# DanEngelbrecht/longtail

Hardware: AMD Instinct MI355X
Metric: ingest GB/s (chunk+hash+compress) (higher is better)
Workload: dtype u8/u32

## Files before the change

longtail_amd/csrc/k_blake3.hip:

```cpp
#include "lthip_internal.h"

#include <stdlib.h>

namespace
{

enum
{
    F_CHUNK_START = 1,
    F_CHUNK_END = 2,
    F_PARENT = 4,
    F_ROOT = 8
};

#define B3_IV0 0x6A09E667u
#define B3_IV1 0xBB67AE85u
#define B3_IV2 0x3C6EF372u
#define B3_IV3 0xA54FF53Au
#define B3_IV4 0x510E527Fu
#define B3_IV5 0x9B05688Cu
#define B3_IV6 0x1F83D9ABu
#define B3_IV7 0x5BE0CD19u

__device__ __forceinline__ uint32_t rotr32(uint32_t x, uint32_t r) { return __builtin_amdgcn_alignbit(x, x, r); }

__device__ __forceinline__ void b3_g(uint32_t& a, uint32_t& b, uint32_t& c, uint32_t& d, uint32_t mx, uint32_t my)
{
    a = a + b + mx;
    d = rotr32(d ^ a, 16);
    c = c + d;
    b = rotr32(b ^ c, 12);
    a = a + b + my;
    d = rotr32(d ^ a, 8);
    c = c + d;
    b = rotr32(b ^ c, 7);
}

#define B3_ROUND(m0, m1, m2, m3, m4, m5, m6, m7, m8, m9, m10, m11, m12, m13, m14, m15) \
    b3_g(s0, s4, s8, s12, m0, m1);                                                      \
    b3_g(s1, s5, s9, s13, m2, m3);                                                      \
    b3_g(s2, s6, s10, s14, m4, m5);                                                     \
    b3_g(s3, s7, s11, s15, m6, m7);                                                     \
    b3_g(s0, s5, s10, s15, m8, m9);                                                     \
    b3_g(s1, s6, s11, s12, m10, m11);                                                   \
    b3_g(s2, s7, s8, s13, m12, m13);                                                    \
    b3_g(s3, s4, s9, s14, m14, m15);

__device__ __forceinline__ void b3_compress(uint32_t (&cv)[8], const uint32_t (&m)[16], uint32_t counter_lo,
                                            uint32_t block_len, uint32_t flags)
{
    uint32_t s0 = cv[0], s1 = cv[1], s2 = cv[2], s3 = cv[3], s4 = cv[4], s5 = cv[5], s6 = cv[6], s7 = cv[7];
    uint32_t s8 = B3_IV0, s9 = B3_IV1, s10 = B3_IV2, s11 = B3_IV3;
    uint32_t s12 = counter_lo, s13 = 0u, s14 = block_len, s15 = flags;
    B3_ROUND(m[0], m[1], m[2], m[3], m[4], m[5], m[6], m[7], m[8], m[9], m[10], m[11], m[12], m[13], m[14], m[15])
    B3_ROUND(m[2], m[6], m[3], m[10], m[7], m[0], m[4], m[13], m[1], m[11], m[12], m[5], m[9], m[14], m[15], m[8])
    B3_ROUND(m[3], m[4], m[10], m[12], m[13], m[2], m[7], m[14], m[6], m[5], m[9], m[0], m[11], m[15], m[8], m[1])
    B3_ROUND(m[10], m[7], m[12], m[9], m[14], m[3], m[13], m[15], m[4], m[0], m[11], m[2], m[5], m[8], m[1], m[6])
    B3_ROUND(m[12], m[13], m[9], m[11], m[15], m[10], m[14], m[8], m[7], m[2], m[5], m[3], m[0], m[1], m[6], m[4])
    B3_ROUND(m[9], m[14], m[11], m[5], m[8], m[12], m[15], m[1], m[13], m[3], m[0], m[10], m[2], m[6], m[4], m[7])
    B3_ROUND(m[11], m[15], m[5], m[0], m[1], m[9], m[8], m[6], m[14], m[10], m[2], m[12], m[3], m[4], m[7], m[13])
    cv[0] = s0 ^ s8;
    cv[1] = s1 ^ s9;
    cv[2] = s2 ^ s10;
    cv[3] = s3 ^ s11;
    cv[4] = s4 ^ s12;
    cv[5] = s5 ^ s13;
    cv[6] = s6 ^ s14;
    cv[7] = s7 ^ s15;
}

typedef uint32_t u32x4_a4 __attribute__((ext_vector_type(4), aligned(4)));

__device__ __forceinline__ uint32_t leaves_of(uint32_t len) { return len ? (len + 1023u) >> 10 : 1u; }

__global__ void k_leaf_counts(const uint32_t* __restrict__ lens, uint64_t bound, const uint32_t* __restrict__ n_dev,
                              uint32_t* __restrict__ counts)
{
    uint64_t i = (uint64_t)blockIdx.x * blockDim.x + threadIdx.x;
    uint64_t n = n_dev ? (*n_dev < bound ? *n_dev : bound) : bound;
    if (i < n)
        counts[i] = leaves_of(lens[i]);
}

#ifndef LTHIP_B3_PW
#define LTHIP_B3_PW 1024
#endif
constexpr int PW = LTHIP_B3_PW;
constexpr int PW_MAXN = 256;
constexpr int PW_SLOTS = PW + PW_MAXN;
#ifndef LTHIP_B3_PW_THREADS
#define LTHIP_B3_PW_THREADS 512
#endif
constexpr int PW_THREADS = LTHIP_B3_PW_THREADS;

__global__ __launch_bounds__(256) void k_blake3_leaves(const uint8_t* __restrict__ data,
                                                       const uint64_t* __restrict__ offsets,
                                                       const uint32_t* __restrict__ lens,
                                                       const uint32_t* __restrict__ leaf_prefix,
                                                       uint64_t count_bound, const uint32_t* __restrict__ n_dev,
                                                       uint32_t* __restrict__ cvs, uint32_t* __restrict__ win_first)
{
    const uint32_t count = (uint32_t)(n_dev ? (*n_dev < count_bound ? *n_dev : count_bound) : count_bound);
    const uint32_t total = leaf_prefix[count];
    const uint64_t g64 = (uint64_t)blockIdx.x * blockDim.x + threadIdx.x;
    if (g64 >= total)
        return;
    const uint32_t g = (uint32_t)g64;
    uint32_t lo = 0, hi = count;
    while (hi - lo > 1)
    {
        const uint32_t mid = lo + ((hi - lo) >> 1);
        if (leaf_prefix[mid] <= g)
            lo = mid;
        else
            hi = mid;
    }
    const uint32_t c = lo;
    const uint32_t first = leaf_prefix[c];
    const uint32_t k = g - first;
    if (win_first && (g & (uint32_t)(PW - 1)) == 0u)
        win_first[g / (uint32_t)PW] = k == 0u ? c : c + 1u;
    const uint32_t rlen = lens[c];
    const uint32_t nleaf = leaves_of(rlen);
    const uint32_t llen = rlen - (k << 10) < 1024u ? rlen - (k << 10) : 1024u;
    const uint8_t* p = data + offsets[c] + ((uint64_t)k << 10);
    const uint32_t root = nleaf == 1u ? (uint32_t)F_ROOT : 0u;

    const uint32_t mis = (uint32_t)((uintptr_t)p & 3u);
    const uint32_t sh = mis * 8u;
    const uint32_t* q = reinterpret_cast<const uint32_t*>(p - mis);

    uint32_t cv[8] = {B3_IV0, B3_IV1, B3_IV2, B3_IV3, B3_IV4, B3_IV5, B3_IV6, B3_IV7};
    const uint32_t nblocks = llen ? (llen + 63u) >> 6 : 1u;

    for (uint32_t b = 0; b + 1 < nblocks; ++b)
    {
        const uint32_t* src = q + b * 16u;
        uint32_t w[17];
        const u32x4_a4 v0 = *reinterpret_cast<const u32x4_a4*>(src);
        const u32x4_a4 v1 = *reinterpret_cast<const u32x4_a4*>(src + 4);
        const u32x4_a4 v2 = *reinterpret_cast<const u32x4_a4*>(src + 8);
        const u32x4_a4 v3 = *reinterpret_cast<const u32x4_a4*>(src + 12);
        w[0] = v0.x; w[1] = v0.y; w[2] = v0.z; w[3] = v0.w;
        w[4] = v1.x; w[5] = v1.y; w[6] = v1.z; w[7] = v1.w;
        w[8] = v2.x; w[9] = v2.y; w[10] = v2.z; w[11] = v2.w;
        w[12] = v3.x; w[13] = v3.y; w[14] = v3.z; w[15] = v3.w;
        w[16] = mis ? src[16] : 0u;
        uint32_t m[16];
#pragma unroll
        for (int i = 0; i < 16; ++i)
            m[i] = __builtin_amdgcn_alignbit(w[i + 1], w[i], sh);
        b3_compress(cv, m, k, 64u, b == 0 ? (uint32_t)F_CHUNK_START : 0u);
    }
    {
        const uint32_t b = nblocks - 1u;
        const uint32_t bl = llen - b * 64u;
        const uint32_t* src = q + b * 16u;
        const uint32_t nd = bl ? (mis + bl + 3u) >> 2 : 0u;
        uint32_t w[17];
#pragma unroll
        for (int i = 0; i < 17; ++i)
            w[i] = (uint32_t)i < nd ? src[i] : 0u;
        uint32_t m[16];
#pragma unroll
        for (int i = 0; i < 16; ++i)
        {
            uint32_t v = __builtin_amdgcn_alignbit(w[i + 1], w[i], sh);
            const int rem = (int)bl - 4 * i;
            if (rem <= 0)
                v = 0u;
            else if (rem < 4)
                v &= (1u << (8 * rem)) - 1u;
            m[i] = v;
        }
        uint32_t fl = (uint32_t)F_CHUNK_END | root;
        if (b == 0)
            fl |= (uint32_t)F_CHUNK_START;
        b3_compress(cv, m, k, bl, fl);
    }
    uint4* out = reinterpret_cast<uint4*>(cvs + (uint64_t)g * 8u);
    out[0] = make_uint4(cv[0], cv[1], cv[2], cv[3]);
    out[1] = make_uint4(cv[4], cv[5], cv[6], cv[7]);
}

__device__ __forceinline__ void b3_parent(uint32_t* __restrict__ left, const uint32_t* __restrict__ right, uint32_t flags)
{
    uint32_t m[16];
    const uint4 a0 = reinterpret_cast<const uint4*>(left)[0], a1 = reinterpret_cast<const uint4*>(left)[1];
    const uint4 b0 = reinterpret_cast<const uint4*>(right)[0], b1 = reinterpret_cast<const uint4*>(right)[1];
    m[0] = a0.x; m[1] = a0.y; m[2] = a0.z; m[3] = a0.w; m[4] = a1.x; m[5] = a1.y; m[6] = a1.z; m[7] = a1.w;
    m[8] = b0.x; m[9] = b0.y; m[10] = b0.z; m[11] = b0.w; m[12] = b1.x; m[13] = b1.y; m[14] = b1.z; m[15] = b1.w;
    uint32_t cv[8] = {B3_IV0, B3_IV1, B3_IV2, B3_IV3, B3_IV4, B3_IV5, B3_IV6, B3_IV7};
    b3_compress(cv, m, 0u, 64u, flags);
    reinterpret_cast<uint4*>(left)[0] = make_uint4(cv[0], cv[1], cv[2], cv[3]);
    reinterpret_cast<uint4*>(left)[1] = make_uint4(cv[4], cv[5], cv[6], cv[7]);
}

#ifdef LTHIP_ABLATIONS
#include "ablations/k_blake3_parents_small.inc"
#endif

constexpr uint32_t B3_ONE_PITCH = 1024u + 4u;
__global__ __launch_bounds__(64) void k_blake3_one(const uint8_t* __restrict__ in, uint32_t len, uint64_t* __restrict__ out)
{
    extern __shared__ __attribute__((aligned(16))) uint32_t s_one[];
    uint32_t* s_cv = s_one;
    uint32_t* s_in = s_one + 64 * 8;
    const uint32_t lane = threadIdx.x;
    const uint32_t nleaf = leaves_of(len);
    {
        const uint32_t nvec = (((uintptr_t)in & 15u) == 0u) ? len >> 4 : 0u;
        const uint4* in4 = reinterpret_cast<const uint4*>(in);
        for (uint32_t v0 = 0; v0 < nvec; v0 += 64u * 8u)
        {
            uint4 q[8];
#pragma unroll
            for (int u = 0; u < 8; ++u)
            {
                const uint32_t v = v0 + (uint32_t)u * 64u + lane;
                q[u] = v < nvec ? in4[v] : make_uint4(0, 0, 0, 0);
            }
#pragma unroll
            for (int u = 0; u < 8; ++u)
            {
                const uint32_t v = v0 + (uint32_t)u * 64u + lane;
                if (v < nvec)
                {
                    uint32_t* d = s_in + (v >> 6) * (B3_ONE_PITCH / 4u) + (v & 63u) * 4u;
                    d[0] = q[u].x;
                    d[1] = q[u].y;
                    d[2] = q[u].z;
                    d[3] = q[u].w;
                }
            }
        }
        for (uint32_t j = (nvec << 4) + lane; j < len; j += 64u)
            reinterpret_cast<uint8_t*>(s_in)[(j >> 10) * B3_ONE_PITCH + (j & 1023u)] = in[j];
    }
    __syncthreads();
    if (lane < nleaf)
    {
        const uint32_t llen = len - (lane << 10) < 1024u ? len - (lane << 10) : 1024u;
        const uint32_t* pw = s_in + lane * (B3_ONE_PITCH / 4u);
        const uint8_t* p = reinterpret_cast<const uint8_t*>(pw);
        const uint32_t nblocks = llen ? (llen + 63u) >> 6 : 1u;
        uint32_t cv[8] = {B3_IV0, B3_IV1, B3_IV2, B3_IV3, B3_IV4, B3_IV5, B3_IV6, B3_IV7};
        for (uint32_t b = 0; b < nblocks; ++b)
        {
            const uint32_t bl = llen - b * 64u < 64u ? llen - b * 64u : 64u;
            uint32_t m[16];
            if (bl == 64u)
            {
#pragma unroll
                for (int i = 0; i < 16; ++i)
                    m[i] = pw[b * 16u + (uint32_t)i];
            }
            else
            {
#pragma unroll
                for (int i = 0; i < 16; ++i)
                    m[i] = 0u;
                for (uint32_t j = 0; j < bl; ++j)
                    m[j >> 2] |= (uint32_t)p[b * 64u + j] << (8u * (j & 3u));
            }
            uint32_t fl = b == 0 ? (uint32_t)F_CHUNK_START : 0u;
            if (b + 1 == nblocks)
                fl |= (uint32_t)F_CHUNK_END | (nleaf == 1u ? (uint32_t)F_ROOT : 0u);
            b3_compress(cv, m, lane, bl, fl);
        }
#pragma unroll
        for (int i = 0; i < 8; ++i)
            s_cv[lane * 8 + i] = cv[i];
    }
    __syncthreads();
    for (uint32_t stride = 1; stride < nleaf; stride <<= 1)
    {
        const uint32_t last = (stride << 1) >= nleaf;
        const uint32_t k = lane * (stride << 1);
        if (k + stride < nleaf)
            b3_parent(s_cv + k * 8u, s_cv + (k + stride) * 8u, (uint32_t)F_PARENT | (last ? (uint32_t)F_ROOT : 0u));
        __syncthreads();
    }
    if (lane == 0)
        *out = (uint64_t)s_cv[0] | ((uint64_t)s_cv[1] << 32);
}

constexpr int B3S_LEAVES = 1024;

__global__ __launch_bounds__(B3S_LEAVES) void k_blake3_stream_batch(const uint8_t* __restrict__ data, uint32_t leaf0,
                                                                      uint32_t* __restrict__ stack, uint32_t depth_in, uint32_t merges)
{
    __shared__ uint32_t s_cv[B3S_LEAVES * 8];
    const uint32_t t = threadIdx.x;
    {
        const uint32_t* p = reinterpret_cast<const uint32_t*>(data) + (size_t)t * 256u;
        uint32_t cv[8] = {B3_IV0, B3_IV1, B3_IV2, B3_IV3, B3_IV4, B3_IV5, B3_IV6, B3_IV7};
        for (uint32_t b = 0; b < 16u; ++b)
        {
            uint32_t m[16];
            const uint4* q = reinterpret_cast<const uint4*>(p + b * 16u);
            const uint4 v0 = q[0], v1 = q[1], v2 = q[2], v3 = q[3];
            m[0] = v0.x; m[1] = v0.y; m[2] = v0.z; m[3] = v0.w; m[4] = v1.x; m[5] = v1.y; m[6] = v1.z; m[7] = v1.w;
            m[8] = v2.x; m[9] = v2.y; m[10] = v2.z; m[11] = v2.w; m[12] = v3.x; m[13] = v3.y; m[14] = v3.z; m[15] = v3.w;
            b3_compress(cv, m, leaf0 + t, 64u, (b == 0 ? (uint32_t)F_CHUNK_START : 0u) | (b == 15u ? (uint32_t)F_CHUNK_END : 0u));
        }
#pragma unroll
        for (int i = 0; i < 8; ++i)
            s_cv[t * 8 + i] = cv[i];
    }
    __syncthreads();
    for (uint32_t stride = 1; stride < (uint32_t)B3S_LEAVES; stride <<= 1)
    {
        if ((t & (2u * stride - 1u)) == 0u)
            b3_parent(s_cv + t * 8u, s_cv + (t + stride) * 8u, (uint32_t)F_PARENT);
        __syncthreads();
    }
    if (t == 0)
    {
        uint32_t depth = depth_in;
        for (int i = 0; i < 8; ++i)
            stack[depth * 8u + i] = s_cv[i];
        ++depth;
        for (uint32_t m = 0; m < merges; ++m)
        {
            b3_parent(stack + (depth - 2u) * 8u, stack + (depth - 1u) * 8u, (uint32_t)F_PARENT);
            --depth;
        }
    }
}

__global__ __launch_bounds__(B3S_LEAVES) void k_blake3_stream_final(const uint8_t* __restrict__ tail, uint32_t tail_len, uint32_t leaf0,
                                                                      const uint32_t* __restrict__ stack, uint32_t depth_in,
                                                                      uint64_t* __restrict__ out)
{
    __shared__ uint32_t s_cv[B3S_LEAVES * 8];
    __shared__ uint32_t s_stack[64 * 8];
    const uint32_t t = threadIdx.x;
    const uint32_t nleaf = tail_len ? (tail_len + 1023u) >> 10 : (leaf0 == 0u ? 1u : 0u);
    const bool single = leaf0 == 0u && nleaf == 1u;
    if (t < nleaf)
    {
        const uint32_t llen = tail_len - (t << 10) < 1024u ? tail_len - (t << 10) : 1024u;
        const uint8_t* p = tail + ((size_t)t << 10);
        const uint32_t nblocks = llen ? (llen + 63u) >> 6 : 1u;
        uint32_t cv[8] = {B3_IV0, B3_IV1, B3_IV2, B3_IV3, B3_IV4, B3_IV5, B3_IV6, B3_IV7};
        for (uint32_t b = 0; b < nblocks; ++b)
        {
            const uint32_t bl = llen - b * 64u < 64u ? llen - b * 64u : 64u;
            uint32_t m[16];
#pragma unroll
            for (int i = 0; i < 16; ++i)
                m[i] = 0u;
            for (uint32_t j = 0; j < bl; ++j)
                m[j >> 2] |= (uint32_t)p[b * 64u + j] << (8u * (j & 3u));
            uint32_t fl = b == 0 ? (uint32_t)F_CHUNK_START : 0u;
            if (b + 1 == nblocks)
                fl |= (uint32_t)F_CHUNK_END | (single ? (uint32_t)F_ROOT : 0u);
            b3_compress(cv, m, leaf0 + t, bl, fl);
        }
#pragma unroll
        for (int i = 0; i < 8; ++i)
            s_cv[t * 8 + i] = cv[i];
    }
    for (uint32_t i = t; i < depth_in * 8u; i += (uint32_t)B3S_LEAVES)
        s_stack[i] = stack[i];
    __syncthreads();
    if (t != 0)
        return;
    if (single)
    {
        *out = (uint64_t)s_cv[0] | ((uint64_t)s_cv[1] << 32);
        return;
    }
    uint32_t depth = depth_in;
    for (uint32_t j = 0; j + 1 < nleaf; ++j)
    {
        for (int i = 0; i < 8; ++i)
            s_stack[depth * 8u + i] = s_cv[j * 8u + i];
        ++depth;
        uint32_t cnt = leaf0 + j + 1u;
        while ((cnt & 1u) == 0u)
        {
            b3_parent(s_stack + (depth - 2u) * 8u, s_stack + (depth - 1u) * 8u, (uint32_t)F_PARENT);
            --depth;
            cnt >>= 1;
        }
    }
    uint32_t* cur = s_cv + (nleaf - 1u) * 8u;
    while (depth > 0u)
    {
        uint32_t* left = s_stack + (depth - 1u) * 8u;
        b3_parent(left, cur, (uint32_t)F_PARENT | (depth == 1u ? (uint32_t)F_ROOT : 0u));
        cur = left;
        --depth;
    }
    *out = (uint64_t)cur[0] | ((uint64_t)cur[1] << 32);
}

__global__ __launch_bounds__(PW_THREADS) void k_blake3_parents_window(const uint32_t* __restrict__ leaf_prefix, uint64_t count_bound,
                                                               const uint32_t* __restrict__ n_dev, const uint32_t* __restrict__ cvs,
                                                               const uint32_t* __restrict__ win_first, uint64_t* __restrict__ hashes)
{
    __shared__ uint4 s_cv[PW_SLOTS * 2];
    __shared__ uint32_t s_info[PW_SLOTS];
    __shared__ uint16_t s_list[PW_SLOTS / 2 + 64];
    __shared__ uint32_t s_cnt, s_maxn;
    const uint32_t count = (uint32_t)(n_dev ? (*n_dev < count_bound ? *n_dev : count_bound) : count_bound);
    const uint32_t total = leaf_prefix[count];
    const uint64_t w0 = (uint64_t)blockIdx.x * PW;
    if (w0 >= total)
        return;
    const int tid = threadIdx.x;
    const int lane = tid & 63;
    const uint32_t c_lo = win_first[blockIdx.x];
    const uint32_t c_hi = w0 + PW >= total ? count : win_first[blockIdx.x + 1u];
    const uint32_t nch = c_hi - c_lo;
    if (nch == 0)
        return;
    const uint32_t wbase = leaf_prefix[c_lo];
    const uint32_t nslots = leaf_prefix[c_hi] - wbase;
    if (tid == 0)
    {
        s_cnt = 0;
        s_maxn = 0;
    }
    {
        const uint4* g = reinterpret_cast<const uint4*>(cvs) + (uint64_t)wbase * 2u;
        for (uint32_t v = tid; v < nslots * 2u; v += PW_THREADS)
            s_cv[v] = g[v];
    }
    __syncthreads();
    if (nch * 8u < nslots)
    {
        for (uint32_t j = tid >> 6; j < nch; j += PW_THREADS / 64)
        {
            const uint32_t p0 = leaf_prefix[c_lo + j], n = leaf_prefix[c_lo + j + 1] - p0;
            for (uint32_t k = lane; k < n; k += 64)
                s_info[p0 - wbase + k] = k | (n << 16);
            if (lane == 0)
                atomicMax(&s_maxn, n);
        }
    }
    else
    {
        for (uint32_t j = tid; j < nch; j += PW_THREADS)
        {
            const uint32_t p0 = leaf_prefix[c_lo + j], n = leaf_prefix[c_lo + j + 1] - p0;
            for (uint32_t k = 0; k < n; ++k)
                s_info[p0 - wbase + k] = k | (n << 16);
            atomicMax(&s_maxn, n);
        }
    }
    __syncthreads();
    const uint32_t maxn = s_maxn;
    uint32_t rot = blockIdx.x;
    for (uint32_t st = 1; st < maxn; st <<= 1, ++rot)
    {
        for (uint32_t s0 = 0; s0 < nslots; s0 += PW_THREADS)
        {
            const uint32_t sl = s0 + (uint32_t)tid;
            const uint32_t info = sl < nslots ? s_info[sl] : 0u;
            const uint32_t k = info & 0xFFFFu, n = info >> 16;
            const bool is = (k & ((st << 1) - 1u)) == 0u && k + st < n;
            const uint64_t mask = __builtin_amdgcn_ballot_w64(is);
            uint32_t base = 0;
            if (lane == 0 && mask)
                base = atomicAdd(&s_cnt, (uint32_t)__builtin_popcountll(mask));
            base = __builtin_amdgcn_readfirstlane(base);
            if (is)
                s_list[base + (uint32_t)__builtin_popcountll(mask & ((1ull << lane) - 1ull))] = (uint16_t)sl;
        }
        __syncthreads();
        const uint32_t nm = s_cnt;
        for (uint32_t mi = ((uint32_t)tid + 64u * rot) & (uint32_t)(PW_THREADS - 1); mi < nm; mi += PW_THREADS)
        {
            const uint32_t sl = s_list[mi];
            const uint32_t n = s_info[sl] >> 16;
            const uint4 a0 = s_cv[2u * sl], a1 = s_cv[2u * sl + 1u];
            const uint4 b0 = s_cv[2u * (sl + st)], b1 = s_cv[2u * (sl + st) + 1u];
            uint32_t m[16] = {a0.x, a0.y, a0.z, a0.w, a1.x, a1.y, a1.z, a1.w, b0.x, b0.y, b0.z, b0.w, b1.x, b1.y, b1.z, b1.w};
            uint32_t cv[8] = {B3_IV0, B3_IV1, B3_IV2, B3_IV3, B3_IV4, B3_IV5, B3_IV6, B3_IV7};
            b3_compress(cv, m, 0u, 64u, (uint32_t)F_PARENT | ((st << 1) >= n ? (uint32_t)F_ROOT : 0u));
            s_cv[2u * sl] = make_uint4(cv[0], cv[1], cv[2], cv[3]);
            s_cv[2u * sl + 1u] = make_uint4(cv[4], cv[5], cv[6], cv[7]);
        }
        __syncthreads();
        if (tid == 0)
            s_cnt = 0;
        __syncthreads();
    }
    for (uint32_t j = tid; j < nch; j += PW_THREADS)
    {
        const uint4 r = s_cv[2u * (leaf_prefix[c_lo + j] - wbase)];
        hashes[c_lo + j] = (uint64_t)r.x | ((uint64_t)r.y << 32);
    }
}

__global__ __launch_bounds__(256) void k_blake3_parents_level(const uint32_t* __restrict__ leaf_prefix, uint32_t count,
                                                              uint32_t stride, uint32_t* __restrict__ cvs)
{
    const uint32_t total = leaf_prefix[count];
    const uint64_t g64 = (uint64_t)blockIdx.x * blockDim.x + threadIdx.x;
    if (g64 >= total)
        return;
    const uint32_t g = (uint32_t)g64;
    uint32_t lo = 0, hi = count;
    while (hi - lo > 1)
    {
        const uint32_t mid = lo + ((hi - lo) >> 1);
        if (leaf_prefix[mid] <= g)
            lo = mid;
        else
            hi = mid;
    }
    const uint32_t slot0 = leaf_prefix[lo];
    const uint32_t n = leaf_prefix[lo + 1] - slot0;
    const uint32_t k = g - slot0;
    if ((k & ((stride << 1) - 1u)) != 0u || k + stride >= n)
        return;
    const uint32_t last = (stride << 1) >= n;
    b3_parent(cvs + (uint64_t)g * 8u, cvs + (uint64_t)(g + stride) * 8u, (uint32_t)F_PARENT | (last ? (uint32_t)F_ROOT : 0u));
}

__global__ void k_blake3_emit(const uint32_t* __restrict__ leaf_prefix, uint32_t count, const uint32_t* __restrict__ cvs,
                              uint64_t* __restrict__ hashes)
{
    const uint64_t c = (uint64_t)blockIdx.x * blockDim.x + threadIdx.x;
    if (c >= count)
        return;
    const uint32_t* base = cvs + (uint64_t)leaf_prefix[c] * 8u;
    hashes[c] = (uint64_t)base[0] | ((uint64_t)base[1] << 32);
}

}

int lthip_launch_blake3(lthip_ctx* ctx, const uint8_t* d_data, const uint64_t* d_offsets, const uint32_t* d_lens,
                        const uint32_t* d_count, uint64_t count_bound, uint64_t leaf_bound, uint64_t max_len,
                        uint64_t* d_hashes)
{
    if (count_bound == 0)
        return 0;
    void *lc, *lp, *cv;
    int err;
    if ((err = lthip_scratch(ctx, S_LEAF_COUNT, (count_bound + 1) * 4, &lc)))
        return err;
    if ((err = lthip_scratch(ctx, S_LEAF_PREFIX, (count_bound + 1) * 4, &lp)))
        return err;
    {
        LaunchTimer t(ctx, LTHIP_K_COMPACT);
        hipLaunchKernelGGL(k_leaf_counts, dim3((uint32_t)div_up_u64(count_bound, 256)), dim3(256), 0, ctx->stream, d_lens,
                           count_bound, d_count, (uint32_t*)lc);
        LTHIP_LAUNCH_CHECK(ctx);
    }
    if ((err = lthip_exclusive_scan_u32(ctx, (const uint32_t*)lc, (uint32_t*)lp, count_bound, d_count, LTHIP_K_COMPACT)))
        return err;

    const bool small_trees = max_len != 0 && max_len <= 256u * 1024u;
    uint32_t host_count = 0;
    if (leaf_bound == 0 || !small_trees)
    {
        if (d_count)
        {
            LTHIP_CHECK(ctx, hipMemcpyAsync(&host_count, d_count, 4, hipMemcpyDeviceToHost, ctx->stream));
            LTHIP_CHECK(ctx, lthip_stream_wait(ctx));
            if (host_count > count_bound)
                host_count = (uint32_t)count_bound;
        }
        else
            host_count = (uint32_t)count_bound;
        uint32_t total = 0;
        LTHIP_CHECK(ctx, hipMemcpyAsync(&total, (const uint32_t*)lp + host_count, 4, hipMemcpyDeviceToHost, ctx->stream));
        LTHIP_CHECK(ctx, lthip_stream_wait(ctx));
        leaf_bound = total;
        if (host_count == 0)
            return 0;
    }
    if (leaf_bound == 0)
        return 0;
    if (leaf_bound > 0xFFFFFFF0ull)
        return lthip_fail(ctx, EINVAL, "blake3", "too many leaves in one batch");
    if ((err = lthip_scratch(ctx, S_CV, leaf_bound * 32, &cv)))
        return err;
    void* wf = nullptr;
    if (small_trees && (err = lthip_scratch(ctx, S_B3_WINDOWS, (leaf_bound / PW + 2) * 4, &wf)))
        return err;
    {
        LaunchTimer t(ctx, LTHIP_K_B3_LEAF);
        LTHIP_ABLATION_ENV(env_pad, "LTHIP_B3_PAD_LDS");
        const int pad_lds = env_pad.get() > 0 ? env_pad.get() : 0;
        hipLaunchKernelGGL(k_blake3_leaves, dim3((uint32_t)div_up_u64(leaf_bound, 256)), dim3(256), (size_t)pad_lds, ctx->stream, d_data,
                           d_offsets, d_lens, (const uint32_t*)lp, count_bound, d_count, (uint32_t*)cv, (uint32_t*)wf);
        LTHIP_LAUNCH_CHECK(ctx);
    }
    if (small_trees)
    {
        LaunchTimer t(ctx, LTHIP_K_B3_PARENT);
#ifdef LTHIP_ABLATIONS
        LTHIP_ABLATION_ENV(env_serial, "LTHIP_B3_SERIAL_PARENTS");
        if (env_serial.get() >= 0)
            hipLaunchKernelGGL(k_blake3_parents_small, dim3((uint32_t)div_up_u64(count_bound, 256)), dim3(256), 0, ctx->stream,
                               d_lens, (const uint32_t*)lp, count_bound, d_count, (uint32_t*)cv, d_hashes);
        else
#endif
            hipLaunchKernelGGL(k_blake3_parents_window, dim3((uint32_t)div_up_u64(leaf_bound, PW)), dim3(PW_THREADS), 0, ctx->stream,
                               (const uint32_t*)lp, count_bound, d_count, (const uint32_t*)cv, (const uint32_t*)wf, d_hashes);
        LTHIP_LAUNCH_CHECK(ctx);
    }
    else
    {
        LaunchTimer t(ctx, LTHIP_K_B3_PARENT);
        uint64_t max_leaves = max_len ? div_up_u64(max_len, 1024) : (1ull << 22);
        for (uint64_t stride = 1; stride < max_leaves; stride <<= 1)
            hipLaunchKernelGGL(k_blake3_parents_level, dim3((uint32_t)div_up_u64(leaf_bound, 256)), dim3(256), 0,
                               ctx->stream, (const uint32_t*)lp, host_count, (uint32_t)stride, (uint32_t*)cv);
        hipLaunchKernelGGL(k_blake3_emit, dim3((uint32_t)div_up_u64(host_count, 256)), dim3(256), 0, ctx->stream,
                           (const uint32_t*)lp, host_count, (const uint32_t*)cv, d_hashes);
        LTHIP_LAUNCH_CHECK(ctx);
    }
    return 0;
}

int lthip_launch_blake3_one(lthip_ctx* ctx, const void* in, uint32_t len, uint64_t* out)
{
    if (len > 65536u)
        return lthip_fail(ctx, EINVAL, "blake3_one", "input above 64 KiB");
    LaunchTimer t(ctx, LTHIP_K_B3_LEAF);
    const size_t lds = 64 * 8 * 4 + (size_t)(len ? (len + 1023u) >> 10 : 1u) * B3_ONE_PITCH;
    if (lds > 64u * 1024u)
    {
        static bool granted[64] = {};
        if (ctx->device < 0 || ctx->device >= 64 || !granted[ctx->device])
        {
            LTHIP_CHECK(ctx, hipFuncSetAttribute(reinterpret_cast<const void*>(&k_blake3_one), hipFuncAttributeMaxDynamicSharedMemorySize, 80 * 1024));
            if (ctx->device >= 0 && ctx->device < 64)
                granted[ctx->device] = true;
        }
    }
    hipLaunchKernelGGL(k_blake3_one, dim3(1), dim3(64), lds, ctx->stream, (const uint8_t*)in, len, out);
    LTHIP_LAUNCH_CHECK(ctx);
    return 0;
}

int lthip_launch_blake3_stream_batch(lthip_ctx* ctx, const void* d_data, uint32_t leaf0, uint32_t* d_stack, uint32_t depth_in, uint32_t merges)
{
    LaunchTimer t(ctx, LTHIP_K_B3_LEAF);
    hipLaunchKernelGGL(k_blake3_stream_batch, dim3(1), dim3(B3S_LEAVES), 0, ctx->stream, (const uint8_t*)d_data, leaf0, d_stack, depth_in, merges);
    LTHIP_LAUNCH_CHECK(ctx);
    return 0;
}

int lthip_launch_blake3_stream_final(lthip_ctx* ctx, const void* d_tail, uint32_t tail_len, uint32_t leaf0, const uint32_t* d_stack,
                                     uint32_t depth, uint64_t* d_out)
{
    LaunchTimer t(ctx, LTHIP_K_B3_PARENT);
    hipLaunchKernelGGL(k_blake3_stream_final, dim3(1), dim3(B3S_LEAVES), 0, ctx->stream, (const uint8_t*)d_tail, tail_len, leaf0, d_stack, depth,
                       d_out);
    LTHIP_LAUNCH_CHECK(ctx);
    return 0;
}
```

longtail_amd/csrc/lz4/lz4_stitch.inc:

```
__device__ __forceinline__ void wg_emit_header(uint8_t* dst, uint32_t lits, uint32_t match_nibble, int tid, int nthreads)
{
    if (tid == 0)
        dst[0] = (uint8_t)(((lits < 15u ? lits : 15u) << 4) | match_nibble);
    if (lits >= 15u)
    {
        const uint32_t len = lits - 15u;
        const uint32_t n = len / 255u + 1u;
        for (uint32_t j = tid; j < n; j += nthreads)
            dst[1 + j] = j + 1 == n ? (uint8_t)(len % 255u) : (uint8_t)255;
    }
}

__global__ __launch_bounds__(64) void k_lz4_stitch_scan(const Lz4Block* __restrict__ blocks, uint32_t b0, uint32_t nblocks, uint32_t SEG,
                                                        const Lz4Meta* __restrict__ meta, Lz4Plan* __restrict__ plan,
                                                        uint32_t* __restrict__ runs, Lz4BlockOut* __restrict__ bout,
                                                        uint32_t* __restrict__ out_sizes, uint8_t* __restrict__ dst, uint32_t spec,
                                                        uint32_t* __restrict__ worklist ,
                                                        uint32_t wl_cap)
{
    const uint32_t b = blockIdx.x + b0;
    if (b >= nblocks)
        return;
    const int lane = threadIdx.x;
    const Lz4Block blk = blocks[b];
    const uint32_t run_base = blk.seg_base + b;
    uint64_t out_pos = 0;
    uint32_t carry = 0;
    uint32_t run = 0;
    Lz4Meta m;
    m.seq_bytes = m.tail_lits = m.first_lit_len = m.first_hdr_bytes = 0;
    if ((uint32_t)lane < blk.nseg)
        m = meta[blk.seg_base + (uint32_t)lane];
    for (uint32_t i0 = 0; i0 < blk.nseg; i0 += 64)
    {
        const uint32_t i = i0 + (uint32_t)lane;
        const Lz4Meta cur = m;
        if (i + 64u < blk.nseg)
            m = meta[blk.seg_base + i + 64u];
        const bool valid = i < blk.nseg;
        const bool has = valid && cur.seq_bytes != 0u;
        const uint32_t seg_len = valid ? (blk.size - i * SEG < SEG ? blk.size - i * SEG : SEG) : 0u;
        uint32_t sv = has ? cur.tail_lits : seg_len;
        uint32_t sf = has ? 1u : 0u;
#pragma unroll
        for (int d = 1; d < 64; d <<= 1)
        {
            const uint32_t pv = __shfl_up(sv, d, 64);
            const uint32_t pf = __shfl_up(sf, d, 64);
            if (lane >= d)
            {
                if (!sf)
                    sv += pv;
                sf |= pf;
            }
        }
        if (!sf)
            sv += carry;
        uint32_t cin = __shfl_up(sv, 1, 64);
        if (lane == 0)
            cin = carry;
        const uint32_t L = cin + cur.first_lit_len;
        const uint32_t hdr = 1u + lz4_len_bytes(L);
        const uint64_t adv = has ? (uint64_t)hdr + L + (cur.seq_bytes - cur.first_hdr_bytes - cur.first_lit_len) : 0ull;
        uint64_t pos = adv;
#pragma unroll
        for (int d = 1; d < 64; d <<= 1)
        {
            const uint64_t pv = __shfl_up(pos, d, 64);
            if (lane >= d)
                pos += pv;
        }
        const uint64_t my_pos = out_pos + pos - adv;
        const uint64_t hm = __builtin_amdgcn_ballot_w64(has);
        const uint32_t before = (uint32_t)__builtin_popcountll(hm & ((1ull << lane) - 1ull));
        Lz4Plan pl;
        pl.hdr_pos = 0xFFFFFFFFu;
        pl.hdr_lits = pl.first_lit_dst = pl.body_dst = 0;
        pl.tail_rel = cin;
        pl.run = run_base + run + before;
        if (has)
        {
            const uint64_t lit_dst = my_pos + hdr;
            runs[run_base + run + before] = (uint32_t)lit_dst;
            pl.hdr_pos = (uint32_t)my_pos;
            pl.hdr_lits = L;
            pl.first_lit_dst = (uint32_t)(lit_dst + cin);
            pl.body_dst = pl.first_lit_dst + cur.first_lit_len;
            pl.tail_rel = 0;
            pl.run = run_base + run + before + 1u;
        }
        if (valid)
            plan[blk.seg_base + i] = pl;
        out_pos += __shfl(pos, 63, 64);
        carry = __shfl(sv, 63, 64);
        run += (uint32_t)__builtin_popcountll(hm);
    }
    const uint32_t hdr = 1u + lz4_len_bytes(carry);
    const uint64_t lit_dst = out_pos + hdr;
    const uint64_t total = lit_dst + carry;
    if (total <= (uint64_t)blk.dst_cap)
    {
        if (run == 0u && spec)
        {
            if (blk.nseg)
                wg_emit_header(dst + blk.dst_off + out_pos, carry, 0u, lane, 64);
        }
        else
        {
            uint32_t base = 0;
            if (lane == 0)
                base = atomicAdd(worklist, blk.ngrp);
            base = __builtin_amdgcn_readfirstlane(base);
            for (uint32_t k = lane; k < blk.ngrp; k += 64)
            {
                worklist[1u + base + k] = blk.grp_base + k;
                worklist[1u + wl_cap + base + k] = b;
            }
        }
    }
    if (lane == 0)
    {
        runs[run_base + run] = (uint32_t)lit_dst;
        Lz4BlockOut bo;
        bo.final_hdr_pos = (uint32_t)out_pos;
        bo.final_lits = carry;
        bo.total = total <= (uint64_t)blk.dst_cap ? (uint32_t)total : 0u;
        bo.pad = run == 0u ? 1u : 0u;
        bout[b] = bo;
        out_sizes[b] = bo.total;
    }
}

__device__ __forceinline__ void wg_copy(uint8_t* __restrict__ dst, const uint8_t* __restrict__ src, uint32_t n, int tid,
                                        int nthreads)
{
    if (n == 0)
        return;
    uint32_t head = (uint32_t)((16u - ((uintptr_t)dst & 15u)) & 15u);
    if (head > n)
        head = n;
    if ((uint32_t)tid < head)
        dst[tid] = src[tid];
    dst += head;
    src += head;
    n -= head;
    const uint32_t nvec = n >> 4;
    const uint32_t mis = (uint32_t)((uintptr_t)src & 3u);
    const uint32_t sh = mis * 8u;
    const uint32_t* s4 = reinterpret_cast<const uint32_t*>(src - mis);
    for (uint32_t v = tid; v < nvec; v += nthreads)
    {
        const uint32_t* q = s4 + v * 4u;
        const u32x4_a4 a = *reinterpret_cast<const u32x4_a4*>(q);
        const uint32_t e = mis ? q[4] : 0u;
        uint4 o;
        o.x = __builtin_amdgcn_alignbit(a.y, a.x, sh);
        o.y = __builtin_amdgcn_alignbit(a.z, a.y, sh);
        o.z = __builtin_amdgcn_alignbit(a.w, a.z, sh);
        o.w = __builtin_amdgcn_alignbit(e, a.w, sh);
        *reinterpret_cast<uint4*>(dst + (uint64_t)v * 16u) = o;
    }
    const uint32_t done = nvec << 4;
    if ((uint32_t)tid < n - done)
        dst[done + tid] = src[done + tid];
}


constexpr int K6_THREADS = 256;

#ifdef LTHIP_K6_WAVES
__attribute__((amdgpu_waves_per_eu(LTHIP_K6_WAVES, LTHIP_K6_WAVES)))
#endif
__global__ __launch_bounds__(K6_THREADS) void k_lz4_stitch_copy(const uint8_t* __restrict__ src,
                                                                 const Lz4Block* __restrict__ blocks, uint32_t nblocks,
                                                                 uint32_t SEG, const uint8_t* __restrict__ streams,
                                                                 const Lz4Meta* __restrict__ meta,
                                                                 const Lz4Plan* __restrict__ plan,
                                                                 const uint32_t* __restrict__ runs,
                                                                 const Lz4BlockOut* __restrict__ bout,
                                                                 uint8_t* __restrict__ dst, const uint32_t* __restrict__ worklist,
                                                                 uint32_t gunits , uint32_t wl_cap)
{
    const int tid = threadIdx.x;
    const uint32_t nwork = worklist[0];
    (void)nblocks;
  for (uint32_t wi = blockIdx.x; wi < nwork; wi += gridDim.x)
  {
    const uint32_t grp = worklist[1u + wi];
    const uint32_t lo = worklist[1u + wl_cap + wi];
    const Lz4Block blk = blocks[lo];
    const Lz4BlockOut bo = bout[lo];
    uint8_t* d = dst + blk.dst_off;
    const uint32_t i0 = (grp - blk.grp_base) * gunits;
    const uint32_t i1 = i0 + gunits < blk.nseg ? i0 + gunits : blk.nseg;
    const int lane = tid & 63;
    for (uint32_t i = i0 + (uint32_t)(tid >> 6); i < i1; i += K6_THREADS / 64)
    {
        const uint32_t seg = blk.seg_base + i;
        const uint32_t seg_start = i * SEG;
        const uint32_t len = blk.size - seg_start < SEG ? blk.size - seg_start : SEG;
        const Lz4Meta m = meta[seg];
        const Lz4Plan pl = plan[seg];
        const uint8_t* s = src + blk.src_off + seg_start;
        const uint8_t* stream = streams + (uint64_t)seg * lz4_stream_stride(SEG);
        uint32_t tail = len;
        if (m.seq_bytes)
        {
            wg_emit_header(d + pl.hdr_pos, pl.hdr_lits, stream[0] & 15u, lane, 64);
            wg_copy(d + pl.first_lit_dst, s, m.first_lit_len, lane, 64);
            const uint32_t skip = m.first_hdr_bytes + m.first_lit_len;
            wg_copy(d + pl.body_dst, stream + skip, m.seq_bytes - skip, lane, 64);
            tail = m.tail_lits;
        }
        wg_copy(d + runs[pl.run] + pl.tail_rel, s + (len - tail), tail, lane, 64);
        if (i + 1 == blk.nseg)
            wg_emit_header(d + bo.final_hdr_pos, bo.final_lits, 0u, lane, 64);
    }
  }
}

__global__ void k_lz4_empty_blocks(const Lz4Block* __restrict__ blocks, uint32_t nblocks,
                                   const Lz4BlockOut* __restrict__ bout, uint8_t* __restrict__ dst)
{
    const uint32_t b = blockIdx.x * blockDim.x + threadIdx.x;
    if (b >= nblocks)
        return;
    if (blocks[b].nseg == 0 && bout[b].total == 1)
        dst[blocks[b].dst_off] = 0;
}
```

Before: 888.6.

## Precompute per-level BLAKE3 merge lists and fast-path incompressible LZ4 blocks

The windowed BLAKE3 parent-reduction kernel now builds, in one pass, a list of all merges for every tree level. It uses per-thread counts, a DPP wave prefix sum and a cross-wave sum, so the per-level ballot/atomic list rebuild and its extra barriers go away. Merge counts are capped at 8 levels packed into 16-bit fields, which limits window size and chunk leaf counts. Separately, the LZ4 stitch-scan kernel gets a fast path: when no segment in a block produced any sequences, it writes a single literal-run header and finishes early instead of running the full scan.

```diff
diff --git a/longtail_amd/csrc/k_blake3.hip b/longtail_amd/csrc/k_blake3.hip
--- a/longtail_amd/csrc/k_blake3.hip
+++ b/longtail_amd/csrc/k_blake3.hip
@@ -397,14 +397,59 @@
     *out = (uint64_t)cur[0] | ((uint64_t)cur[1] << 32);
 }
 
+constexpr int PW_LEVELS = 8;
+
+struct PwCounts
+{
+    uint32_t w[PW_LEVELS / 2];
+};
+__device__ __forceinline__ uint32_t pw_field(const PwCounts& c, uint32_t lvl) { return (c.w[lvl >> 1] >> (16u * (lvl & 1u))) & 0xFFFFu; }
+
+__device__ __forceinline__ uint32_t pw_merges(uint32_t n, uint32_t lvl)
+{
+    const uint32_t st = 1u << lvl;
+    return n > st ? (n + st - 1u) >> (lvl + 1u) : 0u;
+}
+__device__ __forceinline__ void pw_add_range(PwCounts& c, uint32_t n)
+{
+#pragma unroll
+    for (uint32_t l = 0; l < (uint32_t)PW_LEVELS; ++l)
+        c.w[l >> 1] += pw_merges(n, l) << (16u * (l & 1u));
+}
+
+__device__ __forceinline__ uint32_t wave_prefix_sum(uint32_t x)
+{
+    x += (uint32_t)__builtin_amdgcn_update_dpp(0, (int)x, 0x111, 0xF, 0xF, true);
+    x += (uint32_t)__builtin_amdgcn_update_dpp(0, (int)x, 0x112, 0xF, 0xF, true);
+    x += (uint32_t)__builtin_amdgcn_update_dpp(0, (int)x, 0x114, 0xF, 0xF, true);
+    x += (uint32_t)__builtin_amdgcn_update_dpp(0, (int)x, 0x118, 0xF, 0xF, true);
+    x += (uint32_t)__builtin_amdgcn_update_dpp(0, (int)x, 0x142, 0xA, 0xF, true);
+    x += (uint32_t)__builtin_amdgcn_update_dpp(0, (int)x, 0x143, 0xC, 0xF, true);
+    return x;
+}
+
+__device__ __forceinline__ void pw_merge(uint4* __restrict__ s_cv, uint32_t entry, uint32_t st)
+{
+    const uint32_t sl = entry & 0x7FFFu;
+    const uint4 a0 = s_cv[2u * sl], a1 = s_cv[2u * sl + 1u];
+    const uint4 b0 = s_cv[2u * (sl + st)], b1 = s_cv[2u * (sl + st) + 1u];
+    uint32_t m[16] = {a0.x, a0.y, a0.z, a0.w, a1.x, a1.y, a1.z, a1.w, b0.x, b0.y, b0.z, b0.w, b1.x, b1.y, b1.z, b1.w};
+    uint32_t cv[8] = {B3_IV0, B3_IV1, B3_IV2, B3_IV3, B3_IV4, B3_IV5, B3_IV6, B3_IV7};
+    b3_compress(cv, m, 0u, 64u, (uint32_t)F_PARENT | ((entry & 0x8000u) ? (uint32_t)F_ROOT : 0u));
+    s_cv[2u * sl] = make_uint4(cv[0], cv[1], cv[2], cv[3]);
+    s_cv[2u * sl + 1u] = make_uint4(cv[4], cv[5], cv[6], cv[7]);
+}
+
 __global__ __launch_bounds__(PW_THREADS) void k_blake3_parents_window(const uint32_t* __restrict__ leaf_prefix, uint64_t count_bound,
                                                                const uint32_t* __restrict__ n_dev, const uint32_t* __restrict__ cvs,
                                                                const uint32_t* __restrict__ win_first, uint64_t* __restrict__ hashes)
 {
+    static_assert(PW_SLOTS < 0x8000, "a list entry is a slot and the ROOT bit");
+    constexpr int NW = PW_THREADS / 64;
     __shared__ uint4 s_cv[PW_SLOTS * 2];
-    __shared__ uint32_t s_info[PW_SLOTS];
-    __shared__ uint16_t s_list[PW_SLOTS / 2 + 64];
-    __shared__ uint32_t s_cnt, s_maxn;
+    __shared__ uint16_t s_list[PW_SLOTS];
+    __shared__ uint16_t s_p0[PW];
+    __shared__ PwCounts s_wsum[NW];
     const uint32_t count = (uint32_t)(n_dev ? (*n_dev < count_bound ? *n_dev : count_bound) : count_bound);
     const uint32_t total = leaf_prefix[count];
     const uint64_t w0 = (uint64_t)blockIdx.x * PW;
@@ -412,6 +457,7 @@
         return;
     const int tid = threadIdx.x;
     const int lane = tid & 63;
+    const int wave = tid >> 6;
     const uint32_t c_lo = win_first[blockIdx.x];
     const uint32_t c_hi = w0 + PW >= total ? count : win_first[blockIdx.x + 1u];
     const uint32_t nch = c_hi - c_lo;
@@ -419,79 +465,94 @@
         return;
     const uint32_t wbase = leaf_prefix[c_lo];
     const uint32_t nslots = leaf_prefix[c_hi] - wbase;
-    if (tid == 0)
-    {
-        s_cnt = 0;
-        s_maxn = 0;
-    }
+    const uint32_t rpt = (nch + (uint32_t)PW_THREADS - 1u) / (uint32_t)PW_THREADS;
+    const uint32_t j0 = (uint32_t)tid * rpt < nch ? (uint32_t)tid * rpt : nch;
+    const uint32_t j1 = j0 + rpt < nch ? j0 + rpt : nch;
+    const uint32_t first_p0 = j0 < j1 ? leaf_prefix[c_lo + j0] : 0u;
+    const uint32_t first_p1 = j0 < j1 ? leaf_prefix[c_lo + j0 + 1u] : 0u;
     {
         const uint4* g = reinterpret_cast<const uint4*>(cvs) + (uint64_t)wbase * 2u;
         for (uint32_t v = tid; v < nslots * 2u; v += PW_THREADS)
             s_cv[v] = g[v];
     }
+    PwCounts own = {};
+    {
+        uint32_t p0 = first_p0, p1 = first_p1;
+        for (uint32_t j = j0; j < j1; ++j)
+        {
+            pw_add_range(own, p1 - p0);
+            p0 = p1;
+            if (j + 1u < j1)
+                p1 = leaf_prefix[c_lo + j + 2u];
+        }
+    }
+    PwCounts pre;
+#pragma unroll
+    for (int i = 0; i < PW_LEVELS / 2; ++i)
+    {
+        const uint32_t inc = wave_prefix_sum(own.w[i]);
+        pre.w[i] = inc - own.w[i];
+        if (lane == 63)
+            s_wsum[wave].w[i] = inc;
+    }
     __syncthreads();
-    if (nch * 8u < nslots)
-    {
-        for (uint32_t j = tid >> 6; j < nch; j += PW_THREADS / 64)
-        {
-            const uint32_t p0 = leaf_prefix[c_lo + j], n = leaf_prefix[c_lo + j + 1] - p0;
-            for (uint32_t k = lane; k < n; k += 64)
-                s_info[p0 - wbase + k] = k | (n << 16);
-            if (lane == 0)
-                atomicMax(&s_maxn, n);
-        }
-    }
-    else
-    {
-        for (uint32_t j = tid; j < nch; j += PW_THREADS)
-        {
-            const uint32_t p0 = leaf_prefix[c_lo + j], n = leaf_prefix[c_lo + j + 1] - p0;
-            for (uint32_t k = 0; k < n; ++k)
-                s_info[p0 - wbase + k] = k | (n << 16);
-            atomicMax(&s_maxn, n);
+    PwCounts tot = {};
+#pragma unroll
+    for (int w = 0; w < NW; ++w)
+    {
+#pragma unroll
+        for (int i = 0; i < PW_LEVELS / 2; ++i)
+        {
+            const uint32_t a = s_wsum[w].w[i];
+            tot.w[i] += a;
+            if (w < wave)
+                pre.w[i] += a;
+        }
+    }
+#pragma unroll
+    for (int i = 0; i < PW_LEVELS / 2; ++i)
+        tot.w[i] = __builtin_amdgcn_readfirstlane(tot.w[i]);
+    {
+        uint32_t p0 = first_p0, p1 = first_p1;
+        for (uint32_t j = j0; j < j1; ++j)
+        {
+            const uint32_t n = p1 - p0;
+            const uint32_t slot0 = p0 - wbase;
+            s_p0[j] = (uint16_t)slot0;
+            uint32_t lbase = 0;
+#pragma unroll
+            for (uint32_t l = 0; l < (uint32_t)PW_LEVELS; ++l)
+            {
+                const uint32_t nm = pw_merges(n, l);
+                const uint32_t at = lbase + pw_field(pre, l);
+                const uint32_t root = (2u << l) >= n ? 0x8000u : 0u;
+                for (uint32_t q = 0; q < nm; ++q)
+                    s_list[at + q] = (uint16_t)((slot0 + (q << (l + 1u))) | root);
+                lbase += pw_field(tot, l);
+            }
+            pw_add_range(pre, n);
+            p0 = p1;
+            if (j + 1u < j1)
+                p1 = leaf_prefix[c_lo + j + 2u];
         }
     }
     __syncthreads();
-    const uint32_t maxn = s_maxn;
+    const uint64_t tot_lo = (uint64_t)tot.w[0] | ((uint64_t)tot.w[1] << 32), tot_hi = (uint64_t)tot.w[2] | ((uint64_t)tot.w[3] << 32);
     uint32_t rot = blockIdx.x;
-    for (uint32_t st = 1; st < maxn; st <<= 1, ++rot)
-    {
-        for (uint32_t s0 = 0; s0 < nslots; s0 += PW_THREADS)
-        {
-            const uint32_t sl = s0 + (uint32_t)tid;
-            const uint32_t info = sl < nslots ? s_info[sl] : 0u;
-            const uint32_t k = info & 0xFFFFu, n = info >> 16;
-            const bool is = (k & ((st << 1) - 1u)) == 0u && k + st < n;
-            const uint64_t mask = __builtin_amdgcn_ballot_w64(is);
-            uint32_t base = 0;
-            if (lane == 0 && mask)
-                base = atomicAdd(&s_cnt, (uint32_t)__builtin_popcountll(mask));
-            base = __builtin_amdgcn_readfirstlane(base);
-            if (is)
-                s_list[base + (uint32_t)__builtin_popcountll(mask & ((1ull << lane) - 1ull))] = (uint16_t)sl;
-        }
+    uint32_t off = 0;
+    for (uint32_t lvl = 0; lvl < (uint32_t)PW_LEVELS; ++lvl, ++rot)
+    {
+        const uint32_t nm = (uint32_t)((lvl < 4u ? tot_lo : tot_hi) >> (16u * (lvl & 3u))) & 0xFFFFu;
+        if (nm == 0u)
+            break;
+        for (uint32_t mi = ((uint32_t)tid + 64u * rot) & (uint32_t)(PW_THREADS - 1); mi < nm; mi += PW_THREADS)
+            pw_merge(s_cv, s_list[off + mi], 1u << lvl);
+        off += nm;
         __syncthreads();
-        const uint32_t nm = s_cnt;
-        for (uint32_t mi = ((uint32_t)tid + 64u * rot) & (uint32_t)(PW_THREADS - 1); mi < nm; mi += PW_THREADS)
-        {
-            const uint32_t sl = s_list[mi];
-            const uint32_t n = s_info[sl] >> 16;
-            const uint4 a0 = s_cv[2u * sl], a1 = s_cv[2u * sl + 1u];
-            const uint4 b0 = s_cv[2u * (sl + st)], b1 = s_cv[2u * (sl + st) + 1u];
-            uint32_t m[16] = {a0.x, a0.y, a0.z, a0.w, a1.x, a1.y, a1.z, a1.w, b0.x, b0.y, b0.z, b0.w, b1.x, b1.y, b1.z, b1.w};
-            uint32_t cv[8] = {B3_IV0, B3_IV1, B3_IV2, B3_IV3, B3_IV4, B3_IV5, B3_IV6, B3_IV7};
-            b3_compress(cv, m, 0u, 64u, (uint32_t)F_PARENT | ((st << 1) >= n ? (uint32_t)F_ROOT : 0u));
-            s_cv[2u * sl] = make_uint4(cv[0], cv[1], cv[2], cv[3]);
-            s_cv[2u * sl + 1u] = make_uint4(cv[4], cv[5], cv[6], cv[7]);
-        }
-        __syncthreads();
-        if (tid == 0)
-            s_cnt = 0;
-        __syncthreads();
     }
     for (uint32_t j = tid; j < nch; j += PW_THREADS)
     {
-        const uint4 r = s_cv[2u * (leaf_prefix[c_lo + j] - wbase)];
+        const uint4 r = s_cv[2u * s_p0[j]];
         hashes[c_lo + j] = (uint64_t)r.x | ((uint64_t)r.y << 32);
     }
 }
diff --git a/longtail_amd/csrc/lz4/lz4_stitch.inc b/longtail_amd/csrc/lz4/lz4_stitch.inc
--- a/longtail_amd/csrc/lz4/lz4_stitch.inc
+++ b/longtail_amd/csrc/lz4/lz4_stitch.inc
@@ -24,6 +24,33 @@
     const int lane = threadIdx.x;
     const Lz4Block blk = blocks[b];
     const uint32_t run_base = blk.seg_base + b;
+    if (spec)
+    {
+        uint32_t any = 0;
+#pragma unroll 8
+        for (uint32_t i = (uint32_t)lane; i < blk.nseg; i += 64u)
+            any |= meta[blk.seg_base + i].seq_bytes;
+        if (__builtin_amdgcn_ballot_w64(any != 0u) == 0ull)
+        {
+            const uint32_t lit_dst = 1u + lz4_len_bytes(blk.size);
+            const uint64_t total = (uint64_t)lit_dst + blk.size;
+            const bool fits = total <= (uint64_t)blk.dst_cap;
+            if (fits && blk.nseg)
+                wg_emit_header(dst + blk.dst_off, blk.size, 0u, lane, 64);
+            if (lane == 0)
+            {
+                runs[run_base] = lit_dst;
+                Lz4BlockOut bo;
+                bo.final_hdr_pos = 0u;
+                bo.final_lits = blk.size;
+                bo.total = fits ? (uint32_t)total : 0u;
+                bo.pad = 1u;
+                bout[b] = bo;
+                out_sizes[b] = bo.total;
+            }
+            return;
+        }
+    }
     uint64_t out_pos = 0;
     uint32_t carry = 0;
     uint32_t run = 0;
```

Measured after the change: 877.1. 1.3% lower.
